# xuqingkuang/FluidFramework

Measured on AMD Instinct MI355X. Metric: sequenced merge-tree ops applied/sec (node) at 100K docs; % HBM roofline, higher is better.
Workload: dtype int32; 1 GPU; C3: 100000 docs/GPU x 32 clients x 1024 sequenced ops/doc (BASELINE.json configs[2]), full merge-tree apply incl. zamboni; docs_total=100000, docs_per_gpu=100000, docs_rank0=100000, ops_per_doc=1024, ops_per_launch=32, parallelism=hash-routed docs x1 (splitmix64(docId) mod 1; no collective in apply), comm=LocalComm

## Files before the change

fluidframework_amd/build.py:

```python
import os
import subprocess
import sys

HERE = os.path.dirname(os.path.abspath(__file__))
CSRC = os.path.join(HERE, 'csrc')
LIB = os.path.join(HERE, 'libmtgpu.so')
SOURCES = ['mt_apply.hip', 'mt_apply_reg.hip', 'mt_service.hip', 'mt_refs.hip', 'mt_deli.hip', 'mt_engine.cpp',
           'mt_comm.cpp']
HEADERS = ['mt_state.h', 'mt_wave.h', 'mt_checksum.h', 'mt_synth.h', '../../include/mtgpu.h']
HIPCC = os.environ.get('HIPCC', '/opt/rocm/bin/hipcc')
ARCH = os.environ.get('PYTORCH_ROCM_ARCH', 'gfx950')


def needs_build():
    if not os.path.exists(LIB):
        return True
    t = os.path.getmtime(LIB)
    return any(os.path.getmtime(os.path.join(CSRC, f)) > t for f in SOURCES + HEADERS
               if os.path.exists(os.path.join(CSRC, f)))


def build(force=False, verbose=False, prof=False):
    lib = LIB.replace('libmtgpu.so', 'libmtgpu_prof.so') if prof else LIB
    if not prof and not force and not needs_build():
# ... 66 lines not shown
```

fluidframework_amd/csrc/mt_apply_reg.hip:

```cpp
#include <hip/hip_runtime.h>
#include <stdint.h>

#include "../../include/mtgpu.h"
#include "mt_state.h"
#include "mt_wave.h"

namespace mtr {

constexpr int kMaxNodes = 8;
constexpr int kTextGranularity = 256;
constexpr int kNarrowClients = 32;
constexpr int kC64Clients = 63;
constexpr uint32_t kLenBits = 17;
constexpr uint32_t kLenMask = (1u << kLenBits) - 1;
constexpr uint32_t kNoId = 0x7FFFu;
constexpr uint32_t kEmptyLi = kNoId << kLenBits;
constexpr uint32_t F_RM = (uint32_t)MT_SF_REMOVED << 16;
constexpr uint32_t F_PDEF = (uint32_t)MT_SF_PDEF << 16;
constexpr uint32_t F_NL = (uint32_t)MT_SF_NL << 16;
constexpr uint32_t F_HASNL = (uint32_t)MT_SF_HASNL << 16;
constexpr uint32_t F_MARKER = (uint32_t)MT_SF_MARKER << 16;
constexpr uint32_t F_NLQ = 1u << 21;
constexpr uint32_t kEmptyCf = 0xFFu;
constexpr uint16_t kDead = 0xFFFFu;

#define MT_GLOB __attribute__((address_space(1)))
#define MT_KARG __attribute__((address_space(4)))
template <class T>
MT_DEV MT_GLOB T* gp(T* p) { return (MT_GLOB T*)p; }
typedef const MT_KARG mt_gstate KGState;
typedef uint32_t EvWords __attribute__((ext_vector_type(4)));
MT_DEV void put_event(MT_GLOB mt_event* p, int32_t seq, int op, unsigned flags, int leaf, int pos, uint32_t len,
                      uint32_t pmask = 0, uint32_t pv01 = 0, uint32_t pv23 = 0, uint32_t pv45 = 0, uint32_t pv67 = 0) {
    static_assert(sizeof(mt_event) == 96 && offsetof(mt_event, pvals) == 24, "mt_event");
    MT_GLOB EvWords* q = reinterpret_cast<MT_GLOB EvWords*>(p);
    const EvWords z = {0u, 0u, 0u, 0u};
    q[0] = EvWords{(uint32_t)seq, ((uint32_t)op & 0xFFu) | ((flags & 0xFFu) << 8), (uint32_t)leaf, (uint32_t)pos};
    q[1] = EvWords{len, pmask, pv01, pv23};
// ... 50 lines not shown
    union {
        int32_t scr[CAP + 1];
        uint32_t tln[CAP + 1];
    };
    int32_t hseq[H];
    uint16_t toff[CAP];
    uint16_t hslot[H];
    uint8_t ibcnt[MT_MAXLEV - 1][IB];
    uint8_t lbsc[LB + 1];
    int32_t nb[MT_MAXLEV];
    uint32_t zr[4 * kMaxNodes];
    uint64_t dum[64];
};

struct Elem {
    int32_t seq, rseq;
    uint32_t li, cf, ov, oh;
    int32_t cum;
};
struct Cut {
    uint32_t lli, lcf, rli;
    int32_t pos;
};

template <int K, bool W = false, bool EV = false>
struct RWave {
    using L = RLds<K>;
    static constexpr int CAP = L::CAP;
    static constexpr uint32_t kAll = (1u << K) - 1u;
    typedef int32_t VI __attribute__((ext_vector_type(K)));
    typedef uint32_t VU __attribute__((ext_vector_type(K)));
    typedef uint32_t U4 __attribute__((ext_vector_type(4)));
    typedef uint32_t U2 __attribute__((ext_vector_type(2)));
    L& s;
    const int lane;
    uint8_t* const abase;
    const uint32_t textcap;

    VI seq, rseq;
    VU li, cf, ov;
    VU oh;
    VI cum;
    int ns, nlive, nb0, nlev, heap_n, cur_seq, min_seq, err, err_seq, next_id;
    uint32_t text_top, text_half;
    bool dirty;
    uint32_t pb;
    uint32_t bsm, lvm, sc0, sc1;
    MT_GLOB mt_event* evp = nullptr;
    uint32_t evcap = 0;
    int evn = 0;
    int32_t evseq = 0;
#ifdef MT_PROF
    uint64_t prof[P_NSLOT] = {};
#endif

    MT_DEV RWave(L& lds, uint8_t* a, uint32_t tc)
        : s(lds), lane(lane_id()), abase(a), textcap(tc), dirty(false) {}
    MT_DEV uint8_t* arena() const { return abase + (size_t)text_half * textcap; }

    MT_DEV int idx(int j) const { return lane * K + j; }

    MT_DEV void fail(int code, int32_t sq) {
        if (err == 0) {
            err = code;
            err_seq = sq;
        }
    }
    MT_DEV static uint32_t len_of(uint32_t l) { return l & kLenMask; }
    MT_DEV static uint32_t id_of(uint32_t l) { return l >> kLenBits; }

    MT_DEV uint32_t bs_bits() const { return bsm; }
    MT_DEV uint32_t live_bits() const { return lvm; }
    MT_DEV uint32_t kbit(int k) const {
        const int r = k - lane * K;
        return (r >= 0 && r < K) ? (1u << r) : 0u;
    }
    MT_DEV int sc_of(int a) const {
        const int r = uni(a % K);
        return __builtin_amdgcn_readlane((int)(((sc0 >> r) & 1u) | (((sc1 >> r) & 1u) << 1)), a / K);
    }
    MT_DEV void set_sc(int a, int v) {
        const uint32_t b = kbit(a);
        sc0 = (v & 1) ? (sc0 | b) : (sc0 & ~b);
        sc1 = (v & 2) ? (sc1 | b) : (sc1 & ~b);
// ... 78 lines not shown
        if (lane == 0 && evn < (int)evcap) {
            put_event(evp + evn, evseq, op, flags, leaf, pos, len);
        }
        evn = evn + 1;
    }
    MT_DEV int live_before(int k) const { return uni(wave_total(__popc(lvm & below(k)))); }
    MT_DEV int local_before(int k) const {
        const uint32_t m = lvm & below(k);
        int t = 0;
#pragma unroll
        for (int j = 0; j < K; j++) t += (((m >> j) & 1u) && !(cf[j] & F_RM)) ? (int)len_of(li[j]) : 0;
        return uni(wave_total(t));
    }
    MT_DEV void emit_range(bool is_remove, int32_t S, int C, uint32_t tm, uint64_t pclr, uint64_t pset, bool rewrite) {
        uint32_t hm = 0;
#pragma unroll
        for (int j = 0; j < K; j++) {
            const uint32_t f = cf[j];
            const bool hit = ((tm >> j) & 1u) &&
                             (!is_remove || ((f & F_RM) && rseq[j] == S && ((f >> 8) & 0xFFu) == (uint32_t)C));
            hm |= hit ? (1u << j) : 0u;
        }
        const int hc = __popc(hm);
        const int hinc = wave_incl_scan(hc);
        const int total = wave_last(hinc);
        if (total == 0) return emit(is_remove ? MT_EV_REMOVE : MT_EV_ANNOTATE, MT_EVF_FIRST | MT_EVF_EMPTY, -1, -1, 0);
        int ll = 0, lc = 0;
#pragma unroll
        for (int j = 0; j < K; j++) {
            ll += (((lvm >> j) & 1u) && !(cf[j] & F_RM)) ? (int)len_of(li[j]) : 0;
            lc += (lvm >> j) & 1u;
        }
        int pos = wave_incl_scan(ll) - ll, leaf = wave_incl_scan(lc) - lc, idx = evn + hinc - hc;
        uint32_t okeys = 0, onz = 0;
#pragma unroll
// ... 23 lines not shown
                            const uint32_t v0 = ((rep >> (2 * h)) & 1u) ? (uint32_t)(old >> (16 * h)) & 0xFFu : 0u;
                            const uint32_t v1 = ((rep >> (2 * h + 1)) & 1u) ? (uint32_t)(old >> (16 * h + 8)) & 0xFFu : 0u;
                            pw[h] = v0 | (v1 << 16);
                        }
                        put_event(evp + idx, evseq, eop, efl, leaf, pos, len_of(li[j]), pm, pw[0], pw[1], pw[2], pw[3]);
                    }
                }
                idx++;
            }
            pos += (live && !(cf[j] & F_RM)) ? (int)len_of(li[j]) : 0;
            leaf += live ? 1 : 0;
        }
        evn = evn + total;
    }

    MT_DEV Elem get(int k) const {
        const int lk = k / K, jk = uni(k % K);
        Elem r;
        r.seq = __builtin_amdgcn_readlane(seq[jk], lk);
        r.rseq = __builtin_amdgcn_readlane(rseq[jk], lk);
        r.li = (uint32_t)__builtin_amdgcn_readlane((int)li[jk], lk);
        r.cf = (uint32_t)__builtin_amdgcn_readlane((int)cf[jk], lk);
        r.ov = (uint32_t)__builtin_amdgcn_readlane((int)ov[jk], lk);
        if constexpr (W) r.oh = (uint32_t)__builtin_amdgcn_readlane((int)oh[jk], lk);
        r.cum = __builtin_amdgcn_readlane(cum[jk], lk);
        return r;
    }
    MT_DEV uint32_t get_li(int k) const {
        const int jk = uni(k % K);
        return (uint32_t)__builtin_amdgcn_readlane((int)li[jk], k / K);
    }
    MT_DEV void set_li_cf(int k, uint32_t lv, uint32_t cv) {
        const int r = k - lane * K;
#pragma unroll
        for (int j = 0; j < K; j++) {
            li[j] = j == r ? lv : li[j];
            cf[j] = j == r ? cv : cf[j];
        }
    }
    template <bool CUM>
    MT_DEV void shift_in(int p, const Elem& e, bool bs, int scv, bool live, bool dup = false) {
        mask_shift(p, bs, scv, live);
        const int32_t c_seq = shr1(seq[K - 1], 0), c_rseq = shr1(rseq[K - 1], 0);
        const uint32_t c_li = (uint32_t)shr1((int)li[K - 1], 0), c_cf = (uint32_t)shr1((int)cf[K - 1], 0);
        const uint32_t c_ov = (uint32_t)shr1((int)ov[K - 1], 0);
        const uint32_t c_oh = W ? (uint32_t)shr1((int)oh[K - 1], 0) : 0u;
        const int32_t c_cum = CUM ? shr1(cum[K - 1], 0) : 0;
        const int r = p - lane * K;
        const int rq = dup ? r - 1 : r;
        const int ra = dup ? -K - 2 : r;
#pragma unroll
        for (int j = K - 1; j >= 0; j--) {
            const bool mv = j > rq, at = j == ra;
            const int32_t pseq = j ? seq[j - 1] : c_seq, prseq = j ? rseq[j - 1] : c_rseq;
            const uint32_t pli = j ? li[j - 1] : c_li, pcf = j ? cf[j - 1] : c_cf, pov = j ? ov[j - 1] : c_ov;
            seq[j] = mv ? pseq : (at ? e.seq : seq[j]);
            rseq[j] = mv ? prseq : (at ? e.rseq : rseq[j]);
            li[j] = mv ? pli : (at ? e.li : li[j]);
            cf[j] = mv ? pcf : (at ? e.cf : cf[j]);
            ov[j] = mv ? pov : (at ? e.ov : ov[j]);
            if constexpr (W) {
                const uint32_t poh = j ? oh[j - 1] : c_oh;
                oh[j] = mv ? poh : (at ? e.oh : oh[j]);
            }
            if (CUM) {
                const int32_t pcm = j ? cum[j - 1] : c_cum;
                cum[j] = mv ? pcm : (at ? e.cum : cum[j]);
            }
            __builtin_amdgcn_sched_barrier(0);
        }
        ns = ns + 1;
    }
    MT_DEV void patch_cut(int p, const Cut& c) {
        const int r = p - lane * K;
#pragma unroll
        for (int j = 0; j < K; j++) {
            const bool lp = j == r - 1, rp = j == r;
            li[j] = lp ? c.lli : (rp ? c.rli : li[j]);
            cf[j] = lp ? c.lcf : cf[j];
            cum[j] = lp ? c.pos : cum[j];
        }
    }

    MT_DEV int vis(int j, int32_t R, int C) const {
        const uint32_t f = cf[j];
        const bool seen = ((f & 0xFFu) == (uint32_t)C) | (seq[j] <= R);
        const uint32_t ovw = (W && C > kNarrowClients) ? oh[j] : ov[j];
        const bool hid = ((f & F_RM) != 0) & ((((f >> 8) & 0xFFu) == (uint32_t)C) | (((ovw >> ((C - 1) & 31)) & 1u) != 0) |
                                              (rseq[j] <= R));
        return (seen & !hid & (((lvm >> j) & 1u) != 0)) ? (int)len_of(li[j]) : 0;
    }
    MT_DEV int scan(int32_t R, int C) {
        int acc = 0;
#pragma unroll
        for (int j = 0; j < K; j++) {
            acc += vis(j, R, C);
            cum[j] = acc;
        }
        const int incl = wave_incl_scan(acc);
        const int excl = incl - acc;
#pragma unroll
        for (int j = 0; j < K; j++) cum[j] += excl;
        return wave_last(incl);
    }
    MT_DEV int cs0() const { return shr1(cum[K - 1], 0); }

    MT_DEV uint8_t* lvl(int Lv) { return s.ibcnt[Lv - 1]; }
    MT_DEV int nbl(int Lv) const { return uni(s.nb[Lv]); }

    template <class T>
    MT_DEV void lshift_right(T* a, int from, int count_end) {
// ... 359 lines not shown
        hcf = (pcf & ~F_NL) | (lcf & F_NL) | anynl;
    }

    MT_DEV int scour(int a, int e) {
        const uint32_t lb = live_bits() & below(e) & ~below(a);
        const int c = __popc(lb);
        const int incl = wave_incl_scan(c);
        const int rbase = incl - c;
        const int cnt = wave_last(incl);
        if (cnt > kMaxNodes) return fail(MT_DERR_CAPACITY, cur_seq), cnt;
        uint32_t* const dum = reinterpret_cast<uint32_t*>(s.dum) + lane;
#pragma unroll
        for (int j = 0; j < K; j++) {
            const int q = rbase + __popc(lb & ((1u << j) - 1u));
            uint32_t* const z = ((lb >> j) & 1u) ? &s.zr[q] : dum;
            z[0] = (uint32_t)((cf[j] & F_RM) ? rseq[j] : seq[j]);
            z[kMaxNodes] = li[j];
            z[2 * kMaxNodes] = cf[j];
            z[3 * kMaxNodes] = (uint32_t)idx(j);
        }
        wave_sync();
        const bool mine = lane < cnt;
        const int zq = lane & (kMaxNodes - 1);
        const uint32_t r0 = s.zr[zq], r1 = s.zr[kMaxNodes + zq], r2 = s.zr[2 * kMaxNodes + zq],
                       r3 = s.zr[3 * kMaxNodes + zq];
        const int32_t vsq = mine ? (int32_t)r0 : 0;
        const uint32_t vli = mine ? r1 : 0u;
        uint32_t vcf = mine ? r2 : 0u;
        const int vslot = mine ? (int)r3 : 0;
        const uint64_t pr = s.props[mine ? id_of(vli) : 0u];
        const uint64_t vpr = mine ? pr : 0ull;
        if (__ballot(mine && (vcf & F_NLQ))) {
            arena_sync();
            if (mine && (vcf & F_NLQ)) {
                const uint8_t c = arena()[(uint32_t)s.toff[id_of(vli)] + len_of(vli) - 1];
                vcf = (vcf & ~(F_NL | F_NLQ)) | (c == '\n' ? F_NL : 0u);
            }
        }
        const int32_t minSeq = min_seq;
        const bool rm = mine && (vcf & F_RM) != 0;
        const uint32_t ql = len_of(vli);
        const bool elig = mine && !rm && vsq <= minSeq && ql > 0;
        const bool pelig = shr1(elig ? 1 : 0, 0) != 0;
        const uint32_t pcf = (uint32_t)shr1((int)vcf, 0);
        const uint32_t pprl = (uint32_t)shr1((int)(uint32_t)vpr, 0);
        const uint32_t pprh = (uint32_t)shr1((int)(uint32_t)(vpr >> 32), 0);
        const bool a0 = elig && pelig && !((pcf | vcf) & F_MARKER) && !(pcf & F_NL) && ((pcf ^ vcf) & F_PDEF) == 0 && pprl == (uint32_t)vpr &&
                        pprh == (uint32_t)(vpr >> 32);
        const uint32_t a0m = (uint32_t)__ballot(a0);
        uint32_t appm = a0m;
        if (__ballot(a0 && ql > (uint32_t)kTextGranularity)) {
            const uint32_t em = (uint32_t)__ballot(elig);
            uint32_t plen = 0;
            appm = 0;
            for (int q = 0; q < cnt; q++) {
                const uint32_t lq = (uint32_t)__builtin_amdgcn_readlane((int)ql, q);
                if (((a0m >> q) & 1u) && (plen <= (uint32_t)kTextGranularity || lq <= (uint32_t)kTextGranularity)) {
                    appm |= 1u << q;
                    plen += lq;
                } else {
                    plen = ((em >> q) & 1u) ? lq : 0u;
                }
            }
        }
        const uint32_t unlink = (uint32_t)__ballot(rm && vsq <= minSeq) | appm;
        const int kept = cnt - __popc(unlink);
        const uint32_t heads = ~appm & ((1u << (lane & 31)) - 1u);
        const int vtgt = (lane < 32 && ((appm >> lane) & 1u)) ? 31 - __builtin_clz(heads) : -1;
        if constexpr (EV) {
            const bool app = vtgt >= 0;
            const bool tomb = mine && ((unlink >> lane) & 1u) && !app;
            const int kb = lane - __popc(unlink & (lane < 32 ? ((1u << lane) - 1u) : 0xFFFFFFFFu));
            const int nrec = tomb ? 1 : (app ? 2 : 0);
            const int rinc = wave_incl_scan(nrec);
            const int rtot = wave_last(rinc);
            if (rtot) {
                const int st = live_before(a);
                const int ainc = wave_incl_scan(app ? (int)ql : 0);
                const int hp = app ? vtgt : lane;
                const int kbp = __shfl(kb, hp, 64), aincp = __shfl(ainc, hp, 64);
// ... 174 lines not shown
            be = next_start(kl);
        } else {
        int first = 0x7fffffff;
#pragma unroll
        for (int j = K - 1; j >= 0; j--) {
            const int i = idx(j);
            first = ((i < ns) & (cum[j] >= pos)) ? i : first;
        }
        first = first_hit(first);
        if (first == 0x7fffffff) return fail(MT_DERR_INSERT_FAILED, S), -1;
        const int a = block_start(first), e = next_start(first);
        ba = a;
        be = e;
        int best = 0x7fffffff;
        {
            const int cs = cs0();
#pragma unroll
            for (int j = K - 1; j >= 0; j--) {
                const int i = idx(j);
                const int ce = cum[j];
                const int csj = j ? cum[j - 1] : cs;
                const bool rm_before = ((cf[j] & F_RM) != 0) & (rseq[j] <= R);
                const bool h = (((lvm >> j) & 1u) != 0) & (i >= a) & (i < e) &
                               ((ce > pos) | ((ce == pos) & (csj == pos) & !rm_before));
                best = h ? i : best;
            }
        }
        best = first_hit(best);
        k = best != 0x7fffffff ? best : e;
        }
        const int t = alloc_id(S);
        if (t < 0) return -1;
        if (!arena_reserve((uint32_t)tlen, S, t)) return -1;
        const uint32_t top = text_top;
        bool hasnl = false;
        uint8_t* const ar = arena();
        for (int base = 0; base < tlen; base += 64) {
// ... 5 lines not shown
        dirty = true;
        uint32_t fl = (op.flags & MT_F_MARKER) ? F_MARKER
                                               : ((pbyte(pay, tlen - 1) == '\n' ? F_NL : 0u) | (hasnl ? F_HASNL : 0u));
        uint64_t p = 0;
        if (op.flags & MT_F_PROPS) {
            fl |= F_PDEF;
            p = apply_pairs(0, pay, tlen, np);
        }
        if (lane == 0) {
            s.props[t] = p;
            s.toff[t] = (uint16_t)top;
            s.tln[t] = (uint32_t)tlen;
        }
        text_top = top + (uint32_t)tlen;
        wave_sync();
        en.seq = S;
        en.rseq = 0;
        en.li = (uint32_t)tlen | ((uint32_t)t << kLenBits);
        en.cf = (uint32_t)C | fl;
        en.ov = 0;
        en.oh = 0;
        en.cum = pos + tlen;
        return t;
    }

    MT_DEV void range_action(const mt_op_rec op, const uint8_t* pay, int tlen, int np) {
        const int32_t S = op.seq;
        const int C = op.client, start = op.pos1, end = op.pos2;
        const bool is_remove = op.type == MT_OP_REMOVE;
        const bool rewrite = op.flags & MT_F_REWRITE;
        const uint32_t cbit = 1u << ((C - 1) & 31);
        const bool hic = W && C > kNarrowClients;
        uint64_t pclr = 0, pset = 0;
        if (!is_remove) {
            for (int q = 0; q < np; q++) {
                const int k = (int)pbyte(pay, tlen + 2 * q);
                const uint64_t m = 0xFFull << (8 * k);
                pclr |= m;
                pset = (pset & ~m) | ((uint64_t)pbyte(pay, tlen + 2 * q + 1) << (8 * k));
            }
        }
        uint32_t tm = 0;
        {
            int cs = cs0();
#pragma unroll
            for (int j = 0; j < K; j++) {
                const int ce = cum[j];
                tm |= (ce > cs && cs < end && ce > start) ? (1u << j) : 0u;
                cs = ce;
            }
        }
        if (EV && !is_remove) emit_range(false, S, C, tm, pclr, pset, rewrite);
        if (is_remove) {
#pragma unroll
            for (int j = 0; j < K; j++) {
                const bool touched = (tm >> j) & 1u;
                const uint32_t f = cf[j];
                const bool was_rm = (f & F_RM) != 0;
                const bool mark = touched && !was_rm;
                const bool overlap = touched && was_rm;
                ov[j] = (overlap && !hic) ? (ov[j] | cbit) : ov[j];
                if constexpr (W) oh[j] = (overlap && hic) ? (oh[j] | cbit) : oh[j];
                rseq[j] = mark ? S : rseq[j];
                cf[j] = mark ? ((f & ~0xFF00u) | F_RM | ((uint32_t)C << 8)) : f;
            }
        } else {
            uint64_t* const dum = s.dum + lane;
            constexpr int Q = 4;
#pragma unroll
            for (int j0 = 0; j0 < K; j0 += Q) {
                uint64_t* pa[Q];
                uint64_t pv[Q];
#pragma unroll
                for (int q = 0; q < Q; q++) {
                    if (j0 + q < K) {
                        pa[q] = ((tm >> (j0 + q)) & 1u) ? &s.props[id_of(li[j0 + q])] : dum;
                        pv[q] = *pa[q];
                    }
// ... 26 lines not shown
        const uint8_t* pay = payload + op.payload_off;
        const int tlen = (int)op.payload_len - 2 * np;
        const bool noop = MT_OP_IS_NOOP(op);
        if constexpr (EV) evseq = S;
        int bad = 0;
        const bool ins = op.type == MT_OP_INSERT;
        if (!noop) {
            uint32_t kmax = 0;
            if (op.payload_len >= (uint32_t)(2 * np))
                for (int q = 0; q < np; q++) kmax = max(kmax, pbyte(pay, tlen + 2 * q));
            bad = (op.client == 0 || op.client > (W ? kC64Clients : kNarrowClients)) ? MT_DERR_LIMITS
                  : (op.payload_len < (uint32_t)(2 * np) || !MT_OP_NO_TEXT_OK(op)) ? MT_DERR_BAD_OP
                  : (np > 0 && kmax >= MT_MAX_KEYS) ? MT_DERR_LIMITS
                  : (op.pos1 < 0 || (!ins && op.pos2 < 0)) ? MT_DERR_BAD_OP
                  : !(cur_seq < S) ? MT_DERR_SEQ_ORDER
                  : (!(min_seq <= op.msn) || !(op.msn <= S)) ? MT_DERR_MSN_ORDER : 0;
            if (bad) fail(bad, S);
        }
        if (!noop && !bad) {
            PROF_BEGIN(t0, P_SCAN);
            scan(op.ref_seq, op.client);
            PROF_END(prof, P_SCAN, t0);
            const int nsteps = ins ? (tlen > 0 ? 2 : 1) : 2;
            int kl = -1;
#pragma unroll
            for (int step = 0; step < 2 && step < nsteps; step++) {
                PROF_BEGIN2(t1, P_BOUND, P_INSERT);
                const bool placing = ins && step == 1;
                Elem e{};
                Cut cut{};
                int k = 0, ba = 0, be = 0, t = -1;
                bool go;
                if (!placing) {
                    go = split_prep(step == 0 ? op.pos1 : op.pos2, S, cut, k, ba, be);
                    if (go) kl = k - 1;
                } else {
                    t = place_prep(op, pay, tlen, np, e, k, ba, be, uni(kl));
                    go = t >= 0;
                }
                if (go) {
                    k = uni(k);
                    ba = uni(ba);
                    be = uni(be);
                    t = uni(t);
#ifdef MT_UNI_ELEM
                    e.seq = uni(e.seq);
                    e.rseq = uni(e.rseq);
                    e.li = uniu(e.li);
                    e.cf = uniu(e.cf);
                    e.ov = uniu(e.ov);
                    e.oh = uniu(e.oh);
                    e.cum = uni(e.cum);
                    cut.lli = uniu(cut.lli);
                    cut.lcf = uniu(cut.lcf);
                    cut.rli = uniu(cut.rli);
                    cut.pos = uni(cut.pos);
#endif
                    const bool ok = insert_at(k, ba, be, e, S, cut, !placing);
                    if (placing) {
                        PROF_END(prof, P_INSERT, t1);
                    } else {
                        PROF_END(prof, P_BOUND, t1);
// ... 114 lines not shown
                w[2 * j] = x[0];
                w[2 * j + 1] = x[1];
            }
        } else {
#pragma unroll
            for (int c = 0; c < K / 2; c++) {
                const U4 x = reinterpret_cast<const MT_GLOB U4*>(p)[c];
                w[4 * c] = x[0];
                w[4 * c + 1] = x[1];
                w[4 * c + 2] = x[2];
                w[4 * c + 3] = x[3];
            }
        }
    }

    MT_DEV void load(KGState& g, uint32_t d) {
        const MT_GLOB mt_doc_scalars& sc = gp(g.sc)[d];
        const int n = uni(sc.nseg);
        nlev = uni(sc.nlev);
        heap_n = uni(sc.heap_n);
        cur_seq = uni(sc.cur_seq);
        min_seq = uni(sc.min_seq);
        err = uni(sc.err);
        err_seq = uni(sc.err_seq);
        text_top = uniu(sc.text_top);
        text_half = uniu(sc.text_half);
        nb0 = uni(sc.nb[0]);
        next_id = n;
        nlive = n;
        ns = n;
        if constexpr (EV) {
            evp = gp(g.ev) + (size_t)d * g.evcap;
            evcap = g.evcap;
            evn = uni((int)gp(g.evn)[d]);
            evseq = cur_seq;
        }
        const size_t so = (size_t)d * g.segcap;
// ... 74 lines not shown
            int carry = 0;
#pragma unroll
            for (int cc = 0; cc < LBC; cc++) {
                if (cc * 64 < nb0) {
                    const int b = cc * 64 + lane;
                    const int c = b < nb0 ? (int)lbc_[cc] : 0;
                    const int scv = (int)lbs_[cc];
                    const int incl = wave_incl_scan(c) + carry;
                    if (b < nb0 && c > 0) s.scr[incl - c] = 1 | (scv << 1);
                    nempty += __popcll(wave_ballot(b < nb0 && c == 0));
                    carry = wave_last(incl);
                }
            }
        }
        wave_sync();
        bsm = lvm = sc0 = sc1 = 0u;
#pragma unroll
        for (int j = 0; j < K; j++) {
            const bool in = i0 + j < n;
            const int mk = s.scr[i0 + j];
            seq[j] = in ? (int32_t)vsq[j] : 0x7fffffff;
            rseq[j] = in ? (int32_t)vrs[j] : 0;
            li[j] = in ? (vln[j] | ((uint32_t)(i0 + j) << kLenBits)) : kEmptyLi;
            ov[j] = in ? ((ow[2 * j] >> 1) | (ow[2 * j + 1] << 31)) : 0u;
            if constexpr (W) oh[j] = in ? (ow[2 * j + 1] >> 1) : 0u;
            cf[j] = in ? (byte_at(bcw, j) | (byte_at(brw, j) << 8) | ((byte_at(bfw, j) & 0x1Fu) << 16)) : kEmptyCf;
            cum[j] = 0;
            const uint32_t bit = in ? (1u << j) : 0u;
            lvm |= bit;
            bsm |= (mk & 1) ? bit : 0u;
            sc0 |= (mk & 2) ? bit : 0u;
            sc1 |= (mk & 4) ? bit : 0u;
        }
        wave_sync();
#pragma unroll
        for (int j = 0; j < K; j++) s.tln[i0 + j] = vln[j];
        if (nempty) {
            if (ns + nempty > CAP) {
                fail(MT_DERR_CAPACITY, cur_seq);
            } else {
                int carry = 0, placed = 0;
                for (int base = 0; base < nb0; base += 64) {
                    const int b = base + lane;
                    const int c = b < nb0 ? (int)gp(g.lbcnt)[lo + b] : 0;
                    const int scv = b < nb0 ? (int)gp(g.lbscour)[lo + b] : 0;
                    const int incl = wave_incl_scan(c) + carry;
                    uint64_t em = wave_ballot(b < nb0 && c == 0);
                    while (em) {
                        const int fl = first_lane(em);
                        em &= em - 1;
                        Elem ph;
                        ph.seq = 0x7fffffff;
                        ph.rseq = 0;
                        ph.li = kEmptyLi;
                        ph.cf = kEmptyCf;
                        ph.ov = 0;
                        ph.oh = 0;
                        ph.cum = 0;
                        shift_in<false>(__builtin_amdgcn_readlane(incl - c, fl) + placed, ph, true,
                                        __builtin_amdgcn_readlane(scv, fl), false);
                        placed++;
                    }
                    carry = wave_last(incl);
                }
            }
        }
    }

    template <class T, class F>
    MT_DEV void store_field(const T& v, uint32_t lb, int pbase, int nn, F&& put) {
        int32_t* const dum = reinterpret_cast<int32_t*>(s.dum) + lane;
#pragma unroll
        for (int j = 0; j < K; j++)
            *(((lb >> j) & 1u) ? &s.scr[pbase + __popc(lb & ((1u << j) - 1u))] : dum) = (int32_t)v[j];
        wave_sync();
#pragma clang loop unroll(disable) vectorize(disable)
        for (int base = 0; base < nn; base += 256) {
            uint32_t v[4];
#pragma unroll
            for (int q = 0; q < 4; q++) v[q] = (uint32_t)s.scr[min(base + 64 * q + lane, CAP)];
#pragma unroll
// ... 19 lines not shown
                uint32_t at[K];
#pragma unroll
                for (int j = 0; j < K; j++) {
                    const bool on = (q >> j) & 1u;
                    const uint32_t to = s.toff[on ? id_of(li[j]) : 0u];
                    at[j] = on ? to + len_of(li[j]) - 1 : 0u;
                }
                uint32_t ch[K];
#pragma unroll
                for (int j = 0; j < K; j++) ch[j] = arena()[at[j]];
#pragma unroll
                for (int j = 0; j < K; j++)
                    if ((q >> j) & 1u) cf[j] = (cf[j] & ~(F_NL | F_NLQ)) | (ch[j] == '\n' ? F_NL : 0u);
            }
        }
        store_field(seq, lb, pbase, nn, [&](int i, uint32_t v) { gp(g.seq)[so + i] = (int32_t)v; });
        store_field(rseq, lb, pbase, nn, [&](int i, uint32_t v) { gp(g.rseq)[so + i] = (int32_t)v; });
        store_field(ov, lb, pbase, nn, [&](int i, uint32_t v) { gp(g.ovl)[so + i] = (uint64_t)v << 1; });
        if constexpr (W)
            store_field(oh, lb, pbase, nn, [&](int i, uint32_t v) { gp(g.ovl)[so + i] |= (uint64_t)v << 33; });
        store_field(cf, lb, pbase, nn, [&](int i, uint32_t v) {
            gp(g.client)[so + i] = (uint8_t)(v & 0xFFu);
            gp(g.rclient)[so + i] = (uint8_t)((v >> 8) & 0xFFu);
            gp(g.flags)[so + i] = (uint8_t)((v >> 16) & 0x1Fu);
        });
        store_field(li, lb, pbase, nn, [&](int i, uint32_t v) {
            const uint32_t id = id_of(v);
            gp(g.len)[so + i] = len_of(v);
            gp(g.toff)[so + i] = s.toff[id];
            gp(g.props)[so + i] = s.props[id];
        });
        const uint32_t bm = bs_bits();
// ... 80 lines not shown
    r.flags = (uint8_t)(w3 >> 24);
    r.pos1 = __builtin_amdgcn_readlane((int)blk, l + 4);
    r.pos2 = __builtin_amdgcn_readlane((int)blk, l + 5);
    r.payload_off = (uint32_t)__builtin_amdgcn_readlane((int)blk, l + 6);
    r.payload_len = (uint32_t)__builtin_amdgcn_readlane((int)blk, l + 7);
    return r;
}

MT_DEV KGState& kernarg_gstate() {
    KGState* p = (KGState*)__builtin_amdgcn_kernarg_segment_ptr();
    asm volatile("" : "+s"(p));
    return *p;
}

constexpr int wpe_default(int K) {
    return K <= 3 ? 7 : K <= 5 ? 5 : K <= 8 ? 4 : K <= 11 ? 3 : 2;
}
#ifndef MT_WPE_OV
#define MT_WPE_OV {0}
#endif
constexpr int wpe_ov[17] = MT_WPE_OV;
constexpr int wpe(int K) { return K < 17 && wpe_ov[K] > 0 ? wpe_ov[K] : wpe_default(K); }
template <int K, bool W, bool EV>
MT_DEV void reg_apply(uint8_t* text, uint32_t textcap, const mt_op_rec* __restrict__ ops,
                      const uint8_t* __restrict__ payload, const uint32_t* __restrict__ row_ptr,
                      const uint32_t* __restrict__ doc_ids, uint32_t n_docs, uint32_t op_lo, uint32_t op_cnt) {
    extern __shared__ __attribute__((aligned(16))) unsigned char smem[];
    const uint32_t w = blockIdx.x;
    if (w >= n_docs) return;
    const uint32_t d = doc_ids ? doc_ids[w] : w;
    RLds<K>& lds = *reinterpret_cast<RLds<K>*>(smem);
    RWave<K, W, EV> wv(lds, text + (size_t)d * 2 * textcap, textcap);
    const uint32_t r0 = row_ptr[d], r1 = row_ptr[d + 1];
    const uint32_t a = min(r1, r0 + op_lo);
    const uint32_t b = op_cnt ? min(r1, a + op_cnt) : r1;
    if (a >= b) return;
    PROF_BEGIN(tl, P_LOAD);
    wv.load(kernarg_gstate(), d);
    PROF_END(wv.prof, P_LOAD, tl);
    uint32_t blk0 = load_op_block(ops, a, b, wv.lane);
    uint32_t blk1 = load_op_block(ops, a + 8, b, wv.lane);
    uint32_t pb = load_payload(payload, (uint32_t)__builtin_amdgcn_readlane((int)blk0, 6),
                               (uint32_t)__builtin_amdgcn_readlane((int)blk0, 7), wv.lane);
    uint32_t pbn = 0;
    if (a + 1 < b)
        pbn = load_payload(payload, (uint32_t)__builtin_amdgcn_readlane((int)blk0, 14),
                           (uint32_t)__builtin_amdgcn_readlane((int)blk0, 15), wv.lane);
    for (uint32_t i = a; i < b; i++) {
        if (wv.err) break;
        const mt_op_rec op = op_from_block(blk0, (i - a) & 7u);
        wv.pb = pb;
        PROF_BEGIN(top, P_OP);
        wv.apply(op, payload);
        PROF_END(wv.prof, P_OP, top);
// ... 132 lines not shown
```

fluidframework_amd/csrc/mt_service.hip:

```cpp
#include <hip/hip_runtime.h>
#include <stdint.h>

#include "../../include/mtgpu.h"
#include "mt_checksum.h"
#include "mt_state.h"
#include "mt_wave.h"

__global__ void mt_init_kernel(mt_gstate g, uint32_t n_docs) {
    const uint32_t d = blockIdx.x * blockDim.x + threadIdx.x;
    if (d >= n_docs) return;
    mt_doc_scalars sc{};
    sc.nseg = 0;
    sc.nlev = 1;
    sc.nb[0] = 1;
    sc.n_empty = 1;
    sc.win_op = -1;
    sc.label_keys = MT_NO_LABEL_KEYS;
    g.sc[d] = sc;
    g.loc[d].own = -1;
    g.loc[d].glo = g.loc[d].ghi = g.loc[d].stamp = g.loc[d].lseq = g.loc[d].rgn = g.loc[d].rgpn = 0;
    g.lbcnt[(size_t)d * g.lbcap] = 0;
    g.lbscour[(size_t)d * g.lbcap] = MT_SC_UNDEF;
}

// ... 178 lines not shown
        if (a < b && !sc.err) {
            const int nops = (int)(b - a);
            int32_t own = g.loc[d].own;
            const bool needs_lds = (sc.wide & MT_WIDE_LDS) != 0;
            bool c64 = (sc.wide & MT_WIDE_C64) != 0;
            bool wdoc = (sc.wide & MT_WIDE_DOC) != 0;
            const bool wdoc0 = wdoc;
            bool lds_only = false, editing = own >= 0;
            const uint32_t pend = own >= 0 ? g.loc[d].ghi - g.loc[d].glo : 0u;
            uint32_t nloc = 0, nregen = 0;
            bool key16 = false;
            uint32_t nrem_hi = 0;
            unsigned long long ob = 0;
            bool win = ops && sc.win_op == -1 && sc.err == 0;
            int32_t cur = sc.cur_seq, mn = sc.min_seq;
            for (uint32_t i = a; ops && i < b; i++) {
                const mt_op_rec o = ops[i];
                const uint32_t ty = MT_OP_TYPE(o);
                lds_only = lds_only || ty == MT_OP_LOAD;
                editing = editing || (o.seq == -1 && o.type != MT_OP_LOAD);
                nloc += o.seq == -1 ? 1u : 0u;
                nregen += o.seq == MT_SEQ_REGEN ? 1u : 0u;
                ob += 32ull + o.payload_len;
                nrem_hi += (ty == MT_OP_REMOVE && o.client >= MT_MAX_CLIENTS) ? 1u : 0u;
                if (o.type & MT_OP_WIDE) {
                    const uint32_t np = MT_OP_NPAIRS(o);
                    if (np && (!payload || o.payload_len < 3u * np)) {
                        key16 = true;
                    } else {
                        const uint8_t* pp = payload + o.payload_off + (o.payload_len - 3u * np);
                        for (uint32_t q = 0; q < np; q++) key16 = key16 || pp[3 * q] >= 16;
                    }
                }
                if (!wdoc0) {
                    const uint32_t c = o.client;
                    const bool load = ty == MT_OP_LOAD;
                    const uint32_t c0 = load ? MT_LOAD_CLIENT(o) : c, c1 = load ? MT_LOAD_RCLIENT(o) : 0u;
                    const bool has0 = !load || c0 != MT_CLIENT_NONCOLLAB, has1 = load && o.pos2 >= 0;
                    c64 = c64 || (has0 && c0 > 32) || (has1 && c1 > 32);
// ... 51 lines not shown
                        if (sc.nseg + 2 * nops + (int)sc.n_empty + 1 <= cap && sc.nb[0] + 2 * nops + 1 <= lb &&
                            ib_need + nops + 1 <= ib && sc.heap_n + 4 * nops + 16 <= h) {
                            c = k;
                            break;
                        }
                    }
                    c = n_classes + 1 + (c - first_wide);
                    const bool xk = (sc.wide & MT_WIDE_XK) || key16;
                    const bool xo = MT_WIDE_OVN(sc.wide) + nrem_hi > 16u;
                    const uint32_t w0 = g.sc[d].wide;
                    const uint32_t w1 = (w0 & ~MT_WIDE_XO) | (xk ? MT_WIDE_XK : 0u) | (xo ? MT_WIDE_XO : 0u);
                    if (w1 != w0) g.sc[d].wide = w1;
                    if (xk || xo) atomicAdd(&counts[n_buckets + (c - (n_classes + 1))], 1u);
                }
            }
            if (!wdoc && c < first_lds && (needs_lds || c64)) {
                const int lds_base = n_classes + 1 + (n_classes > first_wide ? n_classes - first_wide : 0);
                c = (needs_lds ? lds_base : lds_base + first_lds) + c;
            }
            if (editing) {
                const int cap = classes[4 * cls];
                const int ebase = n_classes + 1 + (n_classes > first_wide ? n_classes - first_wide : 0) + 2 * first_lds;
                c = cap <= 256    ? ebase
                    : cap <= 512  ? ebase + 1
                    : cap <= 1024 ? n_classes
                    : cap <= 2048 ? ebase + 2
                    : cap <= 4096 ? ebase + 3
                                  : ebase + 6;
                if ((sc.wide & MT_WIDE_GROUPS) || pend + nloc + 4u * nregen > 48u)
                    c = cap <= 1024 ? ebase + 4 : cap <= 4096 ? ebase + 5 : ebase + 7;
            }
            if (acc) {
                unsigned long long st = (unsigned long long)MT_SEG_STATE_BYTES * sc.nseg + 2ull * sc.nb[0] +
// ... 546 lines not shown
```

Before: 333.3 million ops/s.

## Pack seq and rseq into one 16-bit-offset register word for wide register classes

For register-resident waves with K above 3, seq and removed-seq are stored as 16-bit offsets from the document's min_seq and packed into one 32-bit register. This saves a vector register per element. Exact values are rebuilt at store time by reloading the original global value when an offset is zero, and a segment origin index is kept in spare cf bits for that purpose. Documents whose sequence window does not fit are routed by the classifier to the LDS path, or fail with a limits error at load. The waves-per-EU default for K=12 is also raised to 3 to use the freed registers.

After: 337.9 million ops/s, median of 6. 1.01x the previous value.

```diff
diff --git a/fluidframework_amd/build.py b/fluidframework_amd/build.py
--- a/fluidframework_amd/build.py
+++ b/fluidframework_amd/build.py
@@ -7,7 +7,7 @@
 LIB = os.path.join(HERE, 'libmtgpu.so')
 SOURCES = ['mt_apply.hip', 'mt_apply_reg.hip', 'mt_service.hip', 'mt_refs.hip', 'mt_deli.hip', 'mt_engine.cpp',
            'mt_comm.cpp']
-HEADERS = ['mt_state.h', 'mt_wave.h', 'mt_checksum.h', 'mt_synth.h', '../../include/mtgpu.h']
+HEADERS = ['mt_state.h', 'mt_wave.h', 'mt_checksum.h', 'mt_synth.h', 'mt_seqwin.h', '../../include/mtgpu.h']
 HIPCC = os.environ.get('HIPCC', '/opt/rocm/bin/hipcc')
 ARCH = os.environ.get('PYTORCH_ROCM_ARCH', 'gfx950')
 
diff --git a/fluidframework_amd/csrc/mt_apply_reg.hip b/fluidframework_amd/csrc/mt_apply_reg.hip
--- a/fluidframework_amd/csrc/mt_apply_reg.hip
+++ b/fluidframework_amd/csrc/mt_apply_reg.hip
@@ -2,6 +2,7 @@
 #include <stdint.h>
 
 #include "../../include/mtgpu.h"
+#include "mt_seqwin.h"
 #include "mt_state.h"
 #include "mt_wave.h"
 
@@ -22,6 +23,7 @@
 constexpr uint32_t F_MARKER = (uint32_t)MT_SF_MARKER << 16;
 constexpr uint32_t F_NLQ = 1u << 21;
 constexpr uint32_t kEmptyCf = 0xFFu;
+constexpr uint32_t kOrgShift = 22;
 constexpr uint16_t kDead = 0xFFFFu;
 
 #define MT_GLOB __attribute__((address_space(1)))
@@ -102,7 +104,8 @@
 };
 
 struct Elem {
-    int32_t seq, rseq;
+    uint32_t sw;
+    uint32_t rsq;
     uint32_t li, cf, ov, oh;
     int32_t cum;
 };
@@ -125,11 +128,14 @@
     uint8_t* const abase;
     const uint32_t textcap;
 
-    VI seq, rseq;
+    static constexpr bool PK = K > MT_SW_EXACT_K;
+    VU sw;
+    VU rsq;
     VU li, cf, ov;
     VU oh;
     VI cum;
     int ns, nlive, nb0, nlev, heap_n, cur_seq, min_seq, err, err_seq, next_id;
+    int32_t base_seq;
     uint32_t text_top, text_half;
     bool dirty;
     uint32_t pb;
@@ -156,6 +162,12 @@
     }
     MT_DEV static uint32_t len_of(uint32_t l) { return l & kLenMask; }
     MT_DEV static uint32_t id_of(uint32_t l) { return l >> kLenBits; }
+    MT_DEV uint32_t lim_of(int32_t R) const { return PK ? mt_sw_lim(R, base_seq) : (uint32_t)R; }
+    MT_DEV uint32_t key_of(int32_t S) const { return PK ? mt_sw_off(S, base_seq) : (uint32_t)S; }
+    MT_DEV static bool key_le(uint32_t a, uint32_t lim) { return PK ? a <= lim : (int32_t)a <= (int32_t)lim; }
+    MT_DEV bool seq_le(int j, uint32_t lim) const { return PK ? mt_sw_seq_le(sw[j], lim) != 0 : (int32_t)sw[j] <= (int32_t)lim; }
+    MT_DEV bool rseq_le(int j, uint32_t lim) const { return PK ? mt_sw_rseq_le(sw[j], lim) != 0 : (int32_t)rsq[j] <= (int32_t)lim; }
+    MT_DEV bool rseq_eq(int j, uint32_t key) const { return PK ? mt_sw_rseq_eq(sw[j], key) != 0 : rsq[j] == key; }
 
     MT_DEV uint32_t bs_bits() const { return bsm; }
     MT_DEV uint32_t live_bits() const { return lvm; }
@@ -264,11 +276,12 @@
     }
     MT_DEV void emit_range(bool is_remove, int32_t S, int C, uint32_t tm, uint64_t pclr, uint64_t pset, bool rewrite) {
         uint32_t hm = 0;
+        const uint32_t dS = key_of(S);
 #pragma unroll
         for (int j = 0; j < K; j++) {
             const uint32_t f = cf[j];
             const bool hit = ((tm >> j) & 1u) &&
-                             (!is_remove || ((f & F_RM) && rseq[j] == S && ((f >> 8) & 0xFFu) == (uint32_t)C));
+                             (!is_remove || ((f & F_RM) && rseq_eq(j, dS) && ((f >> 8) & 0xFFu) == (uint32_t)C));
             hm |= hit ? (1u << j) : 0u;
         }
         const int hc = __popc(hm);
@@ -322,18 +335,6 @@
         evn = evn + total;
     }
 
-    MT_DEV Elem get(int k) const {
-        const int lk = k / K, jk = uni(k % K);
-        Elem r;
-        r.seq = __builtin_amdgcn_readlane(seq[jk], lk);
-        r.rseq = __builtin_amdgcn_readlane(rseq[jk], lk);
-        r.li = (uint32_t)__builtin_amdgcn_readlane((int)li[jk], lk);
-        r.cf = (uint32_t)__builtin_amdgcn_readlane((int)cf[jk], lk);
-        r.ov = (uint32_t)__builtin_amdgcn_readlane((int)ov[jk], lk);
-        if constexpr (W) r.oh = (uint32_t)__builtin_amdgcn_readlane((int)oh[jk], lk);
-        r.cum = __builtin_amdgcn_readlane(cum[jk], lk);
-        return r;
-    }
     MT_DEV uint32_t get_li(int k) const {
         const int jk = uni(k % K);
         return (uint32_t)__builtin_amdgcn_readlane((int)li[jk], k / K);
@@ -349,7 +350,8 @@
     template <bool CUM>
     MT_DEV void shift_in(int p, const Elem& e, bool bs, int scv, bool live, bool dup = false) {
         mask_shift(p, bs, scv, live);
-        const int32_t c_seq = shr1(seq[K - 1], 0), c_rseq = shr1(rseq[K - 1], 0);
+        const uint32_t c_sq = (uint32_t)shr1((int)sw[K - 1], 0);
+        const uint32_t c_rq = PK ? 0u : (uint32_t)shr1((int)rsq[K - 1], 0);
         const uint32_t c_li = (uint32_t)shr1((int)li[K - 1], 0), c_cf = (uint32_t)shr1((int)cf[K - 1], 0);
         const uint32_t c_ov = (uint32_t)shr1((int)ov[K - 1], 0);
         const uint32_t c_oh = W ? (uint32_t)shr1((int)oh[K - 1], 0) : 0u;
@@ -360,10 +362,13 @@
 #pragma unroll
         for (int j = K - 1; j >= 0; j--) {
             const bool mv = j > rq, at = j == ra;
-            const int32_t pseq = j ? seq[j - 1] : c_seq, prseq = j ? rseq[j - 1] : c_rseq;
+            const uint32_t psq = j ? sw[j - 1] : c_sq;
             const uint32_t pli = j ? li[j - 1] : c_li, pcf = j ? cf[j - 1] : c_cf, pov = j ? ov[j - 1] : c_ov;
-            seq[j] = mv ? pseq : (at ? e.seq : seq[j]);
-            rseq[j] = mv ? prseq : (at ? e.rseq : rseq[j]);
+            sw[j] = mv ? psq : (at ? e.sw : sw[j]);
+            if constexpr (!PK) {
+                const uint32_t prq = j ? rsq[j - 1] : c_rq;
+                rsq[j] = mv ? prq : (at ? e.rsq : rsq[j]);
+            }
             li[j] = mv ? pli : (at ? e.li : li[j]);
             cf[j] = mv ? pcf : (at ? e.cf : cf[j]);
             ov[j] = mv ? pov : (at ? e.ov : ov[j]);
@@ -390,19 +395,20 @@
         }
     }
 
-    MT_DEV int vis(int j, int32_t R, int C) const {
+    MT_DEV int vis(int j, uint32_t Rw, int C) const {
         const uint32_t f = cf[j];
-        const bool seen = ((f & 0xFFu) == (uint32_t)C) | (seq[j] <= R);
+        const bool seen = ((f & 0xFFu) == (uint32_t)C) | seq_le(j, Rw);
         const uint32_t ovw = (W && C > kNarrowClients) ? oh[j] : ov[j];
         const bool hid = ((f & F_RM) != 0) & ((((f >> 8) & 0xFFu) == (uint32_t)C) | (((ovw >> ((C - 1) & 31)) & 1u) != 0) |
-                                              (rseq[j] <= R));
+                                              rseq_le(j, Rw));
         return (seen & !hid & (((lvm >> j) & 1u) != 0)) ? (int)len_of(li[j]) : 0;
     }
     MT_DEV int scan(int32_t R, int C) {
         int acc = 0;
+        const uint32_t Rw = lim_of(R);
 #pragma unroll
         for (int j = 0; j < K; j++) {
-            acc += vis(j, R, C);
+            acc += vis(j, Rw, C);
             cum[j] = acc;
         }
         const int incl = wave_incl_scan(acc);
@@ -792,7 +798,7 @@
         for (int j = 0; j < K; j++) {
             const int q = rbase + __popc(lb & ((1u << j) - 1u));
             uint32_t* const z = ((lb >> j) & 1u) ? &s.zr[q] : dum;
-            z[0] = (uint32_t)((cf[j] & F_RM) ? rseq[j] : seq[j]);
+            z[0] = PK ? ((cf[j] & F_RM) ? mt_sw_drseq(sw[j]) : mt_sw_dseq(sw[j])) : ((cf[j] & F_RM) ? rsq[j] : sw[j]);
             z[kMaxNodes] = li[j];
             z[2 * kMaxNodes] = cf[j];
             z[3 * kMaxNodes] = (uint32_t)idx(j);
@@ -802,7 +808,7 @@
         const int zq = lane & (kMaxNodes - 1);
         const uint32_t r0 = s.zr[zq], r1 = s.zr[kMaxNodes + zq], r2 = s.zr[2 * kMaxNodes + zq],
                        r3 = s.zr[3 * kMaxNodes + zq];
-        const int32_t vsq = mine ? (int32_t)r0 : 0;
+        const uint32_t vsq = mine ? r0 : 0u;
         const uint32_t vli = mine ? r1 : 0u;
         uint32_t vcf = mine ? r2 : 0u;
         const int vslot = mine ? (int)r3 : 0;
@@ -815,10 +821,10 @@
                 vcf = (vcf & ~(F_NL | F_NLQ)) | (c == '\n' ? F_NL : 0u);
             }
         }
-        const int32_t minSeq = min_seq;
+        const uint32_t minSeq = lim_of(min_seq);
         const bool rm = mine && (vcf & F_RM) != 0;
         const uint32_t ql = len_of(vli);
-        const bool elig = mine && !rm && vsq <= minSeq && ql > 0;
+        const bool elig = mine && !rm && key_le(vsq, minSeq) && ql > 0;
         const bool pelig = shr1(elig ? 1 : 0, 0) != 0;
         const uint32_t pcf = (uint32_t)shr1((int)vcf, 0);
         const uint32_t pprl = (uint32_t)shr1((int)(uint32_t)vpr, 0);
@@ -841,7 +847,7 @@
                 }
             }
         }
-        const uint32_t unlink = (uint32_t)__ballot(rm && vsq <= minSeq) | appm;
+        const uint32_t unlink = (uint32_t)__ballot(rm && key_le(vsq, minSeq)) | appm;
         const int kept = cnt - __popc(unlink);
         const uint32_t heads = ~appm & ((1u << (lane & 31)) - 1u);
         const int vtgt = (lane < 32 && ((appm >> lane) & 1u)) ? 31 - __builtin_clz(heads) : -1;
@@ -1046,13 +1052,14 @@
         be = e;
         int best = 0x7fffffff;
         {
+            const uint32_t Rw = lim_of(R);
             const int cs = cs0();
 #pragma unroll
             for (int j = K - 1; j >= 0; j--) {
                 const int i = idx(j);
                 const int ce = cum[j];
                 const int csj = j ? cum[j - 1] : cs;
-                const bool rm_before = ((cf[j] & F_RM) != 0) & (rseq[j] <= R);
+                const bool rm_before = ((cf[j] & F_RM) != 0) & rseq_le(j, Rw);
                 const bool h = (((lvm >> j) & 1u) != 0) & (i >= a) & (i < e) &
                                ((ce > pos) | ((ce == pos) & (csj == pos) & !rm_before));
                 best = h ? i : best;
@@ -1088,8 +1095,8 @@
         }
         text_top = top + (uint32_t)tlen;
         wave_sync();
-        en.seq = S;
-        en.rseq = 0;
+        en.sw = PK ? mt_sw_pack(mt_sw_off(S, base_seq), 0u) : (uint32_t)S;
+        en.rsq = 0;
         en.li = (uint32_t)tlen | ((uint32_t)t << kLenBits);
         en.cf = (uint32_t)C | fl;
         en.ov = 0;
@@ -1114,6 +1121,7 @@
                 pset = (pset & ~m) | ((uint64_t)pbyte(pay, tlen + 2 * q + 1) << (8 * k));
             }
         }
+        const uint32_t dS = key_of(S);
         uint32_t tm = 0;
         {
             int cs = cs0();
@@ -1135,7 +1143,8 @@
                 const bool overlap = touched && was_rm;
                 ov[j] = (overlap && !hic) ? (ov[j] | cbit) : ov[j];
                 if constexpr (W) oh[j] = (overlap && hic) ? (oh[j] | cbit) : oh[j];
-                rseq[j] = mark ? S : rseq[j];
+                if constexpr (PK) sw[j] = mark ? mt_sw_with_drseq(sw[j], dS) : sw[j];
+                else rsq[j] = mark ? dS : rsq[j];
                 cf[j] = mark ? ((f & ~0xFF00u) | F_RM | ((uint32_t)C << 8)) : f;
             }
         } else {
@@ -1192,7 +1201,8 @@
                   : (np > 0 && kmax >= MT_MAX_KEYS) ? MT_DERR_LIMITS
                   : (op.pos1 < 0 || (!ins && op.pos2 < 0)) ? MT_DERR_BAD_OP
                   : !(cur_seq < S) ? MT_DERR_SEQ_ORDER
-                  : (!(min_seq <= op.msn) || !(op.msn <= S)) ? MT_DERR_MSN_ORDER : 0;
+                  : (!(min_seq <= op.msn) || !(op.msn <= S)) ? MT_DERR_MSN_ORDER
+                  : (PK && !mt_sw_fits(S, op.ref_seq, base_seq)) ? MT_DERR_LIMITS : 0;
             if (bad) fail(bad, S);
         }
         if (!noop && !bad) {
@@ -1222,8 +1232,8 @@
                     be = uni(be);
                     t = uni(t);
 #ifdef MT_UNI_ELEM
-                    e.seq = uni(e.seq);
-                    e.rseq = uni(e.rseq);
+                    e.sw = uniu(e.sw);
+                    e.rsq = uniu(e.rsq);
                     e.li = uniu(e.li);
                     e.cf = uniu(e.cf);
                     e.ov = uniu(e.ov);
@@ -1368,13 +1378,14 @@
         }
     }
 
-    MT_DEV void load(KGState& g, uint32_t d) {
+    MT_DEV bool load(KGState& g, uint32_t d) {
         const MT_GLOB mt_doc_scalars& sc = gp(g.sc)[d];
         const int n = uni(sc.nseg);
         nlev = uni(sc.nlev);
         heap_n = uni(sc.heap_n);
         cur_seq = uni(sc.cur_seq);
         min_seq = uni(sc.min_seq);
+        base_seq = min_seq;
         err = uni(sc.err);
         err_seq = uni(sc.err_seq);
         text_top = uniu(sc.text_top);
@@ -1479,23 +1490,41 @@
             }
         }
         wave_sync();
+        bool wide_sq = false;
         bsm = lvm = sc0 = sc1 = 0u;
 #pragma unroll
         for (int j = 0; j < K; j++) {
             const bool in = i0 + j < n;
+            const bool rmj = (byte_at(bfw, j) & MT_SF_REMOVED) != 0;
             const int mk = s.scr[i0 + j];
-            seq[j] = in ? (int32_t)vsq[j] : 0x7fffffff;
-            rseq[j] = in ? (int32_t)vrs[j] : 0;
+            const uint32_t ds = mt_sw_off((int32_t)vsq[j], base_seq);
+            const uint32_t dr = rmj ? mt_sw_off((int32_t)vrs[j], base_seq) : 0u;
+            if constexpr (PK) {
+                sw[j] = in ? mt_sw_pack(ds, dr) : mt_sw_pack(MT_SW_PAD, 0u);
+                wide_sq |= in & ((ds > MT_SW_MAX) | (dr > MT_SW_MAX));
+            } else {
+                sw[j] = in ? vsq[j] : 0x7fffffffu;
+                rsq[j] = in ? vrs[j] : 0u;
+            }
             li[j] = in ? (vln[j] | ((uint32_t)(i0 + j) << kLenBits)) : kEmptyLi;
             ov[j] = in ? ((ow[2 * j] >> 1) | (ow[2 * j + 1] << 31)) : 0u;
             if constexpr (W) oh[j] = in ? (ow[2 * j + 1] >> 1) : 0u;
-            cf[j] = in ? (byte_at(bcw, j) | (byte_at(brw, j) << 8) | ((byte_at(bfw, j) & 0x1Fu) << 16)) : kEmptyCf;
+            cf[j] = in ? (byte_at(bcw, j) | (byte_at(brw, j) << 8) | ((byte_at(bfw, j) & 0x1Fu) << 16) |
+                          (PK ? (uint32_t)(i0 + j) << kOrgShift : 0u))
+                       : kEmptyCf;
             cum[j] = 0;
             const uint32_t bit = in ? (1u << j) : 0u;
             lvm |= bit;
             bsm |= (mk & 1) ? bit : 0u;
             sc0 |= (mk & 2) ? bit : 0u;
             sc1 |= (mk & 4) ? bit : 0u;
+        }
+        if (__ballot(wide_sq)) {
+            if (lane == 0) {
+                gp(g.sc)[d].err = MT_DERR_LIMITS;
+                gp(g.sc)[d].err_seq = cur_seq;
+            }
+            return false;
         }
         wave_sync();
 #pragma unroll
@@ -1515,8 +1544,8 @@
                         const int fl = first_lane(em);
                         em &= em - 1;
                         Elem ph;
-                        ph.seq = 0x7fffffff;
-                        ph.rseq = 0;
+                        ph.sw = PK ? mt_sw_pack(MT_SW_PAD, 0u) : 0x7fffffffu;
+                        ph.rsq = 0;
                         ph.li = kEmptyLi;
                         ph.cf = kEmptyCf;
                         ph.ov = 0;
@@ -1530,6 +1559,7 @@
                 }
             }
         }
+        return true;
     }
 
     template <class T, class F>
@@ -1579,8 +1609,29 @@
                     if ((q >> j) & 1u) cf[j] = (cf[j] & ~(F_NL | F_NLQ)) | (ch[j] == '\n' ? F_NL : 0u);
             }
         }
-        store_field(seq, lb, pbase, nn, [&](int i, uint32_t v) { gp(g.seq)[so + i] = (int32_t)v; });
-        store_field(rseq, lb, pbase, nn, [&](int i, uint32_t v) { gp(g.rseq)[so + i] = (int32_t)v; });
+        VU xs, xr;
+        if constexpr (PK) {
+            uint32_t as_[K], ar_[K];
+#pragma unroll
+            for (int j = 0; j < K; j++) {
+                const bool on = (lb >> j) & 1u;
+                const uint32_t org = cf[j] >> kOrgShift;
+                const bool ns_ = on && mt_sw_dseq(sw[j]) == 0u;
+                const bool nr_ = on && (cf[j] & F_RM) && mt_sw_drseq(sw[j]) == 0u;
+                as_[j] = (uint32_t)gp(g.seq)[so + (ns_ ? org : 0u)];
+                ar_[j] = (uint32_t)gp(g.rseq)[so + (nr_ ? org : 0u)];
+            }
+#pragma unroll
+            for (int j = 0; j < K; j++) {
+                xs[j] = (uint32_t)mt_sw_exact(mt_sw_dseq(sw[j]), base_seq, (int32_t)as_[j]);
+                xr[j] = (cf[j] & F_RM) ? (uint32_t)mt_sw_exact(mt_sw_drseq(sw[j]), base_seq, (int32_t)ar_[j]) : 0u;
+            }
+        } else {
+            xs = sw;
+            xr = rsq;
+        }
+        store_field(xs, lb, pbase, nn, [&](int i, uint32_t v) { gp(g.seq)[so + i] = (int32_t)v; });
+        store_field(xr, lb, pbase, nn, [&](int i, uint32_t v) { gp(g.rseq)[so + i] = (int32_t)v; });
         store_field(ov, lb, pbase, nn, [&](int i, uint32_t v) { gp(g.ovl)[so + i] = (uint64_t)v << 1; });
         if constexpr (W)
             store_field(oh, lb, pbase, nn, [&](int i, uint32_t v) { gp(g.ovl)[so + i] |= (uint64_t)v << 33; });
@@ -1691,7 +1742,7 @@
 }
 
 constexpr int wpe_default(int K) {
-    return K <= 3 ? 7 : K <= 5 ? 5 : K <= 8 ? 4 : K <= 11 ? 3 : 2;
+    return K <= 3 ? 7 : K <= 5 ? 5 : K <= 8 ? 4 : K <= 12 ? 3 : 2;
 }
 #ifndef MT_WPE_OV
 #define MT_WPE_OV {0}
@@ -1713,8 +1764,9 @@
     const uint32_t b = op_cnt ? min(r1, a + op_cnt) : r1;
     if (a >= b) return;
     PROF_BEGIN(tl, P_LOAD);
-    wv.load(kernarg_gstate(), d);
+    const bool loaded = wv.load(kernarg_gstate(), d);
     PROF_END(wv.prof, P_LOAD, tl);
+    if (!loaded) return;
     uint32_t blk0 = load_op_block(ops, a, b, wv.lane);
     uint32_t blk1 = load_op_block(ops, a + 8, b, wv.lane);
     uint32_t pb = load_payload(payload, (uint32_t)__builtin_amdgcn_readlane((int)blk0, 6),
diff --git a/fluidframework_amd/csrc/mt_seqwin.h b/fluidframework_amd/csrc/mt_seqwin.h
--- /dev/null
+++ b/fluidframework_amd/csrc/mt_seqwin.h
@@ -0,0 +1,35 @@
+#ifndef MT_SEQWIN_H
+#define MT_SEQWIN_H
+#include <stdint.h>
+
+#ifndef MT_HD
+#if defined(__HIPCC__)
+#define MT_HD __host__ __device__
+#else
+#define MT_HD
+#endif
+#endif
+
+#define MT_SW_MAX 0x7FFEu
+#define MT_SW_PAD 0x7FFFu
+#define MT_SW_EXACT_K 3
+
+MT_HD static inline uint32_t mt_sw_off(int32_t v, int32_t B) { return v <= B ? 0u : (uint32_t)v - (uint32_t)B; }
+MT_HD static inline int mt_sw_fits(int32_t s_last, int32_t r_min, int32_t B) {
+    return r_min >= B && (s_last <= B || (uint32_t)s_last - (uint32_t)B <= MT_SW_MAX);
+}
+MT_HD static inline uint32_t mt_sw_pack(uint32_t dseq, uint32_t drseq) { return (dseq << 16) | drseq; }
+MT_HD static inline uint32_t mt_sw_dseq(uint32_t w) { return w >> 16; }
+MT_HD static inline uint32_t mt_sw_drseq(uint32_t w) { return w & 0xFFFFu; }
+MT_HD static inline uint32_t mt_sw_with_drseq(uint32_t w, uint32_t drseq) { return (w & 0xFFFF0000u) | drseq; }
+MT_HD static inline uint32_t mt_sw_lim(int32_t R, int32_t B) {
+    const uint32_t d = (uint32_t)R - (uint32_t)B;
+    return d < MT_SW_MAX ? d : MT_SW_MAX;
+}
+MT_HD static inline int mt_sw_seq_le(uint32_t w, uint32_t lim) { return w < ((lim + 1u) << 16); }
+MT_HD static inline int mt_sw_rseq_le(uint32_t w, uint32_t lim) { return mt_sw_drseq(w) <= lim; }
+MT_HD static inline int mt_sw_rseq_eq(uint32_t w, uint32_t ds) { return mt_sw_drseq(w) == ds; }
+MT_HD static inline int32_t mt_sw_exact(uint32_t d, int32_t B, int32_t at_load) {
+    return d ? (int32_t)((uint32_t)B + d) : at_load;
+}
+#endif
diff --git a/fluidframework_amd/csrc/mt_service.hip b/fluidframework_amd/csrc/mt_service.hip
--- a/fluidframework_amd/csrc/mt_service.hip
+++ b/fluidframework_amd/csrc/mt_service.hip
@@ -3,6 +3,7 @@
 
 #include "../../include/mtgpu.h"
 #include "mt_checksum.h"
+#include "mt_seqwin.h"
 #include "mt_state.h"
 #include "mt_wave.h"
 
@@ -216,6 +217,7 @@
             unsigned long long ob = 0;
             bool win = ops && sc.win_op == -1 && sc.err == 0;
             int32_t cur = sc.cur_seq, mn = sc.min_seq;
+            int32_t s_hi = sc.cur_seq, r_lo = 0x7fffffff;
             for (uint32_t i = a; ops && i < b; i++) {
                 const mt_op_rec o = ops[i];
                 const uint32_t ty = MT_OP_TYPE(o);
@@ -225,6 +227,8 @@
                 nregen += o.seq == MT_SEQ_REGEN ? 1u : 0u;
                 ob += 32ull + o.payload_len;
                 nrem_hi += (ty == MT_OP_REMOVE && o.client >= MT_MAX_CLIENTS) ? 1u : 0u;
+                s_hi = o.seq > s_hi ? o.seq : s_hi;
+                r_lo = (!MT_OP_IS_NOOP(o) && o.ref_seq < r_lo) ? o.ref_seq : r_lo;
                 if (o.type & MT_OP_WIDE) {
                     const uint32_t np = MT_OP_NPAIRS(o);
                     if (np && (!payload || o.payload_len < 3u * np)) {
@@ -306,9 +310,10 @@
                     if (xk || xo) atomicAdd(&counts[n_buckets + (c - (n_classes + 1))], 1u);
                 }
             }
-            if (!wdoc && c < first_lds && (needs_lds || c64)) {
+            const bool off_win = classes[4 * cls] > 64 * MT_SW_EXACT_K && (!ops || !mt_sw_fits(s_hi, r_lo, sc.min_seq));
+            if (!wdoc && c < first_lds && (needs_lds || c64 || off_win)) {
                 const int lds_base = n_classes + 1 + (n_classes > first_wide ? n_classes - first_wide : 0);
-                c = (needs_lds ? lds_base : lds_base + first_lds) + c;
+                c = ((needs_lds || off_win) ? lds_base : lds_base + first_lds) + c;
             }
             if (editing) {
                 const int cap = classes[4 * cls];
```
